# yassram/iterative-closest-point

Measured on AMD Instinct MI355X. Metric: ICP iterations/sec (synthetic 1048576-point pair, C4, exact NN), higher is better.
Workload: dtype f64 (30 exact fp64 grid searches (fp32 screen, candidates decided in fp64: the first from cell seeds, the seeded ones the fused grid iteration nn_grid_iter2_kernel, 75% of its queries kept their correspondence by the exclusion certificate without a walk); fp64 transform and reductions)

## Files before the change

### iterative-closest-point_amd/csrc/icp_grid.hip

```cpp
#include <hip/hip_runtime.h>

#include <algorithm>
#include <cmath>
#include <cstdlib>
#include <string>

#include "icp_canon.h"
#include "icp_device.h"
#include "icp_gridbox.h"
#include "icp_kernels.h"

namespace icp {
namespace {

__device__ __forceinline__ double d64g(double px, double py, double pz, double mx, double my,
                                       double mz)
{
    const double dx = px - mx;
    const double dy = py - my;
    const double dz = pz - mz;
    return (dx * dx + dy * dy) + dz * dz;
}


__global__ __launch_bounds__(kBlock) void grid_keys_kernel(const double *__restrict__ mx, const double *__restrict__ my,
                                                         const double *__restrict__ mz, int nm, GridView gv,
                                                         unsigned *__restrict__ key, int *__restrict__ val)
{
    const int i = blockIdx.x * kBlock + threadIdx.x;
    if (i >= nm) return;
    const int cx = cell1(mx[i], gv.lo[0], gv.inv_h, gv.g[0]);
    const int cy = cell1(my[i], gv.lo[1], gv.inv_h, gv.g[1]);
    const int cz = cell1(mz[i], gv.lo[2], gv.inv_h, gv.g[2]);
    key[i] = (unsigned)((cz * gv.g[1] + cy) * gv.g[0] + cx);
    val[i] = i;
}

__global__ __launch_bounds__(kBlock) void grid_starts_kernel(const unsigned *__restrict__ skey, int nm, int ncell,
                                                           int *__restrict__ start)
{
    const int c = blockIdx.x * kBlock + threadIdx.x;
    if (c > ncell) return;
    int lo = 0, hi = nm;
    while (lo < hi) {
        const int mid = (lo + hi) >> 1;
        if (skey[mid] < (unsigned)c) lo = mid + 1;
        else hi = mid;
    }
    start[c] = lo;
}

__global__ __launch_bounds__(kBlock) void grid_gather_kernel(const double4 *__restrict__ m4, int nm,
                                                           const int *__restrict__ sval, double4 *__restrict__ pts,
                                                           float4 *__restrict__ pts32, double c0, double c1, double c2)
{
    const int k = blockIdx.x * kBlock + threadIdx.x;
    if (k >= nm) return;
    const int i = sval[k];
// ... 438 lines not shown
                    const int r = r0 + u * G;
                    int a = 0, b = 0;
                    int x0 = c0[0], x1 = c1[0];
                    const int cy = c0[1] + r % ny, cz = c0[2] + r / ny;
                    if (r < nrows && (!trim || trim_row(q, best, gv, cy, cz, x0, x1))) {
                        const int row = (cz * gv.g[1] + cy) * gv.g[0];
                        a = gv.start[row + x0];
                        b = gv.start[row + x1 + 1];
                    }
                    k0[u] = a;
                    pre[u + 1] = pre[u] + (b - a);
                }
                const int total = pre[KR];
                for (int f0 = 0; f0 < total; f0 += KU) {
                    int k[KU];
#pragma unroll
                    for (int v = 0; v < KU; ++v) {
                        const int f = f0 + v;
                        int p = k0[0] + f;
#pragma unroll
                        for (int u = 1; u < KR; ++u)
                            if (f >= pre[u]) p = k0[u] + (f - pre[u]);
                        k[v] = f < total ? p : -1;
                    }
                    double4 m[KU];
#pragma unroll
                    for (int v = 0; v < KU; ++v)
                        if (k[v] >= 0) m[v] = gv.pts[k[v]];
#pragma unroll
                    for (int v = 0; v < KU; ++v)
                        if (k[v] >= 0)
                            lex_min_pos(best, bi, bk, d64g(q[0], q[1], q[2], m[v].x, m[v].y, m[v].z), (int)m[v].w,
                                        k[v]);
                }
            }
            group_lex_min_pos<G>(best, bi, bk);
            if (sub == 0) {
                const double4 w = bk >= 0 ? gv.pts[bk] : m4[bi];
                idx[t] = bi;
                yx[t] = w.x;
                yy[t] = w.y;
                yz[t] = w.z;
            }
        }
        const bool far = !ok && sub == 0;
        const int fs = wave_append(far_count, far);
        if (far) {
            far_list[fs] = t;
            far_hint[fs] = h;
        }
    }
}

__device__ __forceinline__ float seeded_bound32(double best, double e)
{
    const double s = sqrt(best) * (1.0 + 0x1.0p-50) + 1.7320508075688774 * e;
    return (float)(s * s * (1.0 + 0x1.0p-20)) * (1.0f + 0x1.0p-22f);
}

template <int G, int KR, int KU>
__global__ __launch_bounds__(kBlock) void nn_grid_seeded32_kernel(
    int n, const double *__restrict__ px, const double *__restrict__ py, const double *__restrict__ pz, GridView gv,
    int budget, const double *__restrict__ seedd, const double4 *__restrict__ m4, int *__restrict__ idx,
    double *__restrict__ yx, double *__restrict__ yy, double *__restrict__ yz, int *far_count,
    int *__restrict__ far_list, int *__restrict__ far_hint, const int *__restrict__ stop, int xcd_remap, int trim)
{
    if (stop && *stop) return;
    const int sub = threadIdx.x & (G - 1);
    const int groups = gridDim.x * (kBlock / G);
    const int bx = xcd_row((int)blockIdx.x, (int)gridDim.x, xcd_remap);
    for (int t = (bx * kBlock + threadIdx.x) / G; t < n; t += groups) {
        const int h = idx[t];
        const double q[3] = {px[t], py[t], pz[t]};
        double best = seedd[t];
        int bi = h, bk = -1, c0[3], c1[3];
        const bool ok = h >= 0 && best == best && best < INFINITY && complete_box(q, best, gv, budget, c0, c1);
        if (ok) {
            const double o0 = q[0] - gv.c32[0], o1 = q[1] - gv.c32[1], o2 = q[2] - gv.c32[2];
            const float q0 = (float)o0, q1 = (float)o1, q2 = (float)o2;
            const double e = std::ldexp(fmax(fabs(o0), fmax(fabs(o1), fabs(o2))), -23) + gv.em32;
            const float T = seeded_bound32(best, e);
            const int ny = c1[1] - c0[1] + 1;
            const int nrows = ny * (c1[2] - c0[2] + 1);
            for (int r0 = sub; r0 < nrows; r0 += KR * G) {
                int k0[KR], pre[KR + 1];
                pre[0] = 0;
#pragma unroll
                for (int u = 0; u < KR; ++u) {
                    const int r = r0 + u * G;
                    int a = 0, b = 0;
                    int x0 = c0[0], x1 = c1[0];
                    const int cy = c0[1] + r % ny, cz = c0[2] + r / ny;
                    if (r < nrows && (!trim || trim_row(q, best, gv, cy, cz, x0, x1))) {
                        const int row = (cz * gv.g[1] + cy) * gv.g[0];
                        a = gv.start[row + x0];
                        b = gv.start[row + x1 + 1];
                    }
                    k0[u] = a;
                    pre[u + 1] = pre[u] + (b - a);
                }
                const int total = pre[KR];
                for (int f0 = 0; f0 < total; f0 += KU) {
                    int k[KU];
#pragma unroll
                    for (int v = 0; v < KU; ++v) {
                        const int f = f0 + v;
                        int p = k0[0] + f;
#pragma unroll
                        for (int u = 1; u < KR; ++u)
                            if (f >= pre[u]) p = k0[u] + (f - pre[u]);
                        k[v] = f < total ? p : -1;
// ... 553 lines not shown
    __syncthreads();
    if (threadIdx.x < kCanonCols) {
        const int k = threadIdx.x;
        double v[4];
#pragma unroll
        for (int j = 0; j < 4; ++j)
            v[j] = H == 1 ? sh[j][k] : 0.0 + (sh[H * j][k] + sh[H * j + H - 1][k]);
        rows[(size_t)k * R + wr] = (v[0] + v[1]) + (v[2] + v[3]);
    }
    __shared__ int s_cnt[2][NW];
    for (int o = 32; o >= 1; o >>= 1) far += __shfl_xor(far, o, 64);
    if (lane == 0) {
        s_cnt[0][wave] = far;
        s_cnt[1][wave] = nbig;
    }
    __syncthreads();
    if (threadIdx.x < 2) {
        int tot = 0;
        for (int w = 0; w < NW; ++w) tot += s_cnt[threadIdx.x][w];
        int *dst = threadIdx.x == 0 ? far_acc : big_count;
        if (tot && dst) atomicAdd(dst, tot);
    }
}

constexpr int kNoBound = (int)0xbf800000u;
constexpr int kIter2Slot = 8;
constexpr int kIter2Tile = kCanonCols * kLeafStride;
static_assert(32 * kIter2Slot + 32 / 2 <= kIter2Tile, "the hand-off slots and the walker list alias the tiles");

#ifndef ICP_ITER2_DBG
#define ICP_ITER2_DBG 0
#endif
#ifndef ICP_ITER2_F64
#define ICP_ITER2_F64 0
#endif
#ifndef ICP_ITER2_KU
#define ICP_ITER2_KU 4
#endif
#ifndef ICP_ITER2_KR
#define ICP_ITER2_KR 3
#endif
#ifndef ICP_ITER2_KCAND
#define ICP_ITER2_KCAND ICP_ITER_KCAND
#endif
#ifndef ICP_ITER2_WAVES
#define ICP_ITER2_WAVES 4
#endif
#ifndef ICP_ITER2_GFLOOR
#define ICP_ITER2_GFLOOR 1
#endif
#ifndef ICP_ITER2_NWG_DEFAULT
#define ICP_ITER2_NWG_DEFAULT 1
#endif
template <int KR, int KU, int CH, int NWG>
__global__ __launch_bounds__(64 * NWG) __attribute__((amdgpu_waves_per_eu(ICP_ITER2_WAVES))) void nn_grid_iter2_kernel(
    int n, double *__restrict__ px, double *__restrict__ py, double *__restrict__ pz, double *__restrict__ yx,
    double *__restrict__ yy, double *__restrict__ yz, int *__restrict__ idx, const IterState *__restrict__ st,
    float4 *__restrict__ p32, GridView gv, int box, int budget, int nm, const double4 *__restrict__ m4,
    double *__restrict__ rows, int *far_acc, double far_d2, int *big_count, int xform, int xcd_l, CertArgs ca,
    unsigned long long *__restrict__ dbg)
{
    static_assert(CH == 1 || CH == 2, "one or two chunks a task");
    constexpr bool kDbg = ICP_ITER2_DBG != 0;
    unsigned long long dcnt[4] = {0, 0, 0, 0};
    static_assert(NWG == 4 || NWG == 1, "a row or a strand a workgroup");
    constexpr int NW = NWG, QL = 2 / CH;
    __shared__ double s_tile[NW][CH * kIter2Tile];
    if (st->done) return;
    const int lane = threadIdx.x & 63, wave = threadIdx.x >> 6, u = lane / QL, sub = lane % QL;
    const int C = canon_chunks((size_t)n), S = canon_strands((size_t)n), R = canon_rows((size_t)n);
    const int s = NWG == 4 ? xcd_row((int)blockIdx.x, R, xcd_l) * 4 + wave
                           : xcd_row((int)blockIdx.x, S, xcd_l > 0 ? 4 * xcd_l : xcd_l);
    const int wr = s >> 2;
    double *const tile = s_tile[wave];
    double *const slots = tile;
    int *const wl = (int *)(tile + 32 * CH * kIter2Slot);
    const bool cert_on = ca.state != nullptr, cert_in = cert_on && ca.valid != 0;
    auto wave_sync = [] {
        __builtin_amdgcn_fence(__ATOMIC_RELEASE, "wavefront");
        __builtin_amdgcn_wave_barrier();
        __builtin_amdgcn_fence(__ATOMIC_ACQUIRE, "wavefront");
    };
    double acc = 0.0;
    int far = 0, nbig = 0, ncert = 0, nwalk = 0;
    auto slot_t = [&](int c, int uu) { return (c + (uu >> 5) * S) * kCanonChunk + (uu & 31); };
    for (int c = s; s < S && c < C; c += CH * S) {
        const int t = slot_t(c, u);
        const bool active = c + (u >> 5) * S < C && t < n;
        if (kDbg) dcnt[0] += 1;
        double q[3] = {0.0, 0.0, 0.0}, y[3] = {0.0, 0.0, 0.0};
        int h = -1;
        int4 cs4 = make_int4(kNoBound, kNoBound, -1, -1);
        double mot = 0.0;
        if (active) {
            const double p0 = px[t], p1 = py[t], p2 = pz[t];
            y[0] = yx[t];
            y[1] = yy[t];
            y[2] = yz[t];
            h = idx[t];
            if (cert_in) cs4 = ca.state[t];
            if (xform) {
                transform_point(st->xf, p0, p1, p2, q[0], q[1], q[2]);
                if (cert_in)
                    mot = (double)(__builtin_amdgcn_sqrtf(__double2float_ru(residual2(p0, p1, p2, q[0], q[1], q[2]))) *
                                   (1.0f + 0x1.0p-21f));
            } else {
                q[0] = p0;
                q[1] = p1;
                q[2] = p2;
            }
        }
        const double e = active ? residual2(y[0], y[1], y[2], q[0], q[1], q[2]) : 0.0;
        if (active && sub == 0 && xform) {
            px[t] = q[0];
            py[t] = q[1];
            pz[t] = q[2];
            if (p32)
                p32[t] = make_float4((float)(q[0] - st->xf.c[0]), (float)(q[1] - st->xf.c[1]), (float)(q[2] - st->xf.c[2]),
                                     0.0f);
        }
        if (active && sub == 0) {
            if (far_d2 >= 0.0) {
                if (xform) far += e > far_d2 ? 1 : 0;
            } else if (!(h >= 0 && e * (gv.inv_h * gv.inv_h) < 2.2)) {
                int b0[3], b1[3];
                far += h >= 0 && e == e && e < INFINITY && complete_box(q, e, gv, box, b0, b1) ? 0 : 1;
            }
        }
        double best = e;
        int bi = h;
        double w[3] = {y[0], y[1], y[2]};
        bool certd = false;
        const float R1 = __int_as_float(cs4.x), R3 = __int_as_float(cs4.y);
        if (cert_in && active && h >= 0 && (R1 > 0.0f || R3 > 0.0f)) {
            const double R1c = ((double)R1 - mot) - (double)R1 * 0x1.0p-48;
            const double R3c = ((double)R3 - mot) - (double)R3 * 0x1.0p-48;
            auto inside = [](double d2, double r) { return r > 0.0 && d2 * (1.0 + 0x1.0p-38) < r * r * (1.0 - 0x1.0p-50); };
            double R1n = R1c;
            int2 pn = make_int2(cs4.z, cs4.w);
            certd = inside(e, R1c);
            if (kDbg && !certd && ca.two && cs4.w >= 0 && R3c > 0.0) dcnt[3] += 1;
            if (!certd && ca.two && cs4.w >= 0 && R3c > 0.0) {
                const double4 r2 = gv.pts[cs4.w];
                const double d2 = d64g(q[0], q[1], q[2], r2.x, r2.y, r2.z);
                const int mi2 = (int)r2.w;
                const bool swap = d2 < e || (d2 == e && (unsigned)mi2 < (unsigned)h);
                const double db = swap ? d2 : e;
                if (inside(db, R3c)) {
                    certd = true;
                    const double lb = fmin(R3c, sqrt(swap ? e : d2) * (1.0 - 0x1.0p-40));
                    if (swap) {
                        best = d2;
                        bi = mi2;
                        w[0] = r2.x;
                        w[1] = r2.y;
                        w[2] = r2.z;
                        R1n = lb;
                        pn = make_int2(cs4.w, cs4.z);
                    } else {
                        R1n = fmax(R1c, lb);
                    }
                }
            }
            if (certd && sub == 0) {
                const int4 ns = make_int4(__float_as_int(R1n > 0.0 ? __double2float_rd(R1n) : -1.0f),
                                          __float_as_int(R3c > 0.0 ? __double2float_rd(R3c) : -1.0f), pn.x, pn.y);
                if (bi != h) {
                    ca.state[t] = ns;
                    idx[t] = bi;
                    yx[t] = w[0];
                    yy[t] = w[1];
                    yz[t] = w[2];
                } else {
                    *(int2 *)&ca.state[t] = make_int2(ns.x, ns.y);
                }
            }
        }
        double *const sl = slots + u * kIter2Slot;
        const bool walker = active && !certd;
        if (walker && sub == 0) {
            sl[0] = q[0];
            sl[1] = q[1];
            sl[2] = q[2];
            sl[3] = best;
            ((int *)(sl + 7))[0] = bi;
            ((int *)(sl + 7))[1] = h;
        }
        if (active && sub == 0) {
            sl[4] = w[0];
            sl[5] = w[1];
            sl[6] = w[2];
        }
        const unsigned long long wm = __ballot(walker && sub == 0);
        ncert += certd && sub == 0 ? 1 : 0;
        nwalk += walker && sub == 0 ? 1 : 0;
        const int nW = __popcll(wm);
        if (walker && sub == 0) wl[__popcll(wm & ((1ull << lane) - 1ull))] = u;
        wave_sync();
        if (kDbg) dcnt[1] += nW;
        for (int b0 = 0; b0 < nW; b0 += 32) {
            if (kDbg) dcnt[2] += 1;
            const int nb = min(32, nW - b0);
            const int lg = nb > 16 ? 1 : nb > 8 ? 2 : nb > 4 ? 3 : nb > 2 ? 4 : nb > 1 ? 5 : 6;
            const int G = ICP_ITER2_GFLOOR ? 64 / nb : 1 << lg;
            const int ginv = (65536 + G - 1) / G;
            const int wi = (lane * ginv) >> 16, ws = lane - wi * G, gbase = wi * G;
            const bool wact = wi < nb;
            const int wu = wl[b0 + (wact ? wi : 0)];
            const double *const ws_sl = slots + wu * kIter2Slot;
            double wq[3], wb = INFINITY;
            int wbi = -1;
            wq[0] = ws_sl[0];
            wq[1] = ws_sl[1];
            wq[2] = ws_sl[2];
            if (wact) {
                wb = ws_sl[3];
                wbi = ((const int *)(ws_sl + 7))[0];
            }
            int c0[3] = {0, 0, 0}, c1[3] = {-1, -1, -1};
            double ew = wb;
            bool ok = false;
            if (wact && wbi >= 0 && wb == wb && wb < INFINITY) {
                if (cert_on) {
                    const double rs = sqrt(wb) + ca.skin;
                    ew = rs * rs;
                    ok = complete_box(wq, ew, gv, box, c0, c1);
                    if (!ok) ew = wb;
                }
                if (!ok) ok = complete_box(wq, ew, gv, box, c0, c1);
            }
            if (wact && ws == 0) slots[wu * kIter2Slot + 3] = ew;
            int bk = -1;
            float a1 = INFINITY, a2 = INFINITY;
            int k1 = -1;
            auto other = [&](float v, int k) {
                const bool lt = v < a1;
                a2 = __builtin_amdgcn_fmed3f(a1, v, a2);
                a1 = lt ? v : a1;
                k1 = lt ? k : k1;
            };
            auto eq_of = [&]() {
                const double o0 = wq[0] - gv.c32[0], o1 = wq[1] - gv.c32[1], o2 = wq[2] - gv.c32[2];
                return std::ldexp(fmax(fabs(o0), fmax(fabs(o1), fabs(o2))), -23) + gv.em32;
            };
            if (ok) {
                const float f0 = (float)(wq[0] - gv.c32[0]), f1 = (float)(wq[1] - gv.c32[1]), f2 = (float)(wq[2] - gv.c32[2]);
                const double eq = eq_of();
                const float T = seeded_bound32(wb, eq);
                const int ny = c1[1] - c0[1] + 1, nrq = ny * (c1[2] - c0[2] + 1);
                constexpr int kCand = ICP_ITER2_KCAND;
                int cand[kCand], nc = 0;
                auto flush = [&]() {
                    double4 r[kCand];
#pragma unroll
                    for (int j = 0; j < kCand; ++j)
                        if (j < nc) r[j] = gv.pts[cand[j]];
#pragma unroll
                    for (int j = 0; j < kCand; ++j) {
                        if (j >= nc) break;
                        const int mi = (int)r[j].w;
                        const double d = d64g(wq[0], wq[1], wq[2], r[j].x, r[j].y, r[j].z);
                        if (d < wb || (d == wb && (unsigned)mi < (unsigned)wbi)) {
                            if (cert_on && bk >= 0) other(__double2float_rd(wb), bk);
                            wb = d;
                            wbi = mi;
                            bk = cand[j];
                        } else if (cert_on) {
                            other(__double2float_rd(d), cand[j]);
                        }
                    }
                    nc = 0;
                };
                auto test = [&](const float4 (&m)[KU], const int (&kk)[KU]) {
                    bool cnd[KU];
                    bool anyc = false;
#pragma unroll
                    for (int v = 0; v < KU; ++v) {
                        const float dx = f0 - m[v].x, dy = f1 - m[v].y, dz = f2 - m[v].z;
                        const float d32 = (dx * dx + dy * dy) + dz * dz;
                        const bool val = kk[v] >= 0, fr = d32 > T;
                        if (cert_on) other(val && fr ? d32 : INFINITY, kk[v]);
                        const bool self = val && !fr && __float_as_int(m[v].w) == wbi;
                        bk = self ? kk[v] : bk;
                        cnd[v] = val && !fr && !self;
                        anyc = anyc || cnd[v];
                    }
                    if (__ballot(anyc)) {
#pragma unroll
                        for (int v = 0; v < KU; ++v)
                            if (cnd[v]) {
                                cand[nc++] = kk[v];
                                if (nc == kCand) flush();
                            }
                    }
                };
                const float inv_ny = 1.0f / (float)ny;
                float tr[3];
#pragma unroll
                for (int a = 0; a < 3; ++a) tr[a] = (float)((wq[a] - gv.lo[a]) * gv.inv_h - (double)c0[a]);
                const float rcf = (float)(sqrt(ew) * gv.inv_h * (1.0 + 0x1.0p-18) +
                                          0x1.0p-20 * (1.0 + fabs((double)tr[0]) + fabs((double)tr[1]) + fabs((double)tr[2])));
                const float rc2 = rcf * rcf, xroom = 0x1.0p-20f * (1.0f + fabsf(tr[0]));
                const float xspan = (float)(c1[0] - c0[0] + 1);
                auto row_run = [&](int r, int &a0, int &a1r) {
                    a0 = 0;
                    a1r = 0;
                    if (r >= nrq) return;
                    const int rz = (int)(((float)r + 0.5f) * inv_ny), ry = r - rz * ny;
                    const int row = ((c0[2] + rz) * gv.g[1] + c0[1] + ry) * gv.g[0];
                    int x0 = c0[0], x1 = c1[0];
                    const float dy = fmaxf(0.0f, fmaxf((float)ry - tr[1], tr[1] - (float)(ry + 1)));
                    const float dz = fmaxf(0.0f, fmaxf((float)rz - tr[2], tr[2] - (float)(rz + 1)));
                    const float rem = rc2 - dy * dy - dz * dz;
                    if (rem < 0.0f) return;
                    const float xw = __builtin_amdgcn_sqrtf(rem) * (1.0f + 0x1.0p-20f) + xroom;
                    x0 = max(x0, c0[0] + (int)floorf(fmaxf(tr[0] - xw, -1.0f)));
                    x1 = min(x1, c0[0] + (int)floorf(fminf(tr[0] + xw, xspan)));
                    if (x0 <= x1) {
                        a0 = gv.start[row + x0];
                        a1r = gv.start[row + x1 + 1];
                    }
                };
                {
                    for (int r0 = ws; r0 < nrq; r0 += KR * G) {
                        int k0[KR], pre[KR + 1];
                        pre[0] = 0;
#pragma unroll
                        for (int v = 0; v < KR; ++v) {
                            int a0, a1r;
                            row_run(r0 + v * G, a0, a1r);
                            k0[v] = a0;
                            pre[v + 1] = pre[v] + (a1r - a0);
                        }
                        const int tot = pre[KR];
                        for (int f0 = 0; f0 < tot; f0 += KU) {
                            int kk[KU];
#pragma unroll
                            for (int v = 0; v < KU; ++v) {
                                const int f = f0 + v;
                                int pp = k0[0] + f;
#pragma unroll
                                for (int x = 1; x < KR; ++x)
                                    if (f >= pre[x]) pp = k0[x] + (f - pre[x]);
                                kk[v] = f < tot ? pp : -1;
                            }
                            if constexpr (ICP_ITER2_F64) {
                                double4 mm[KU];
#pragma unroll
                                for (int v = 0; v < KU; ++v) mm[v] = gv.pts[kk[v] >= 0 ? kk[v] : 0];
#pragma unroll
                                for (int v = 0; v < KU; ++v) {
                                    const double d = d64g(wq[0], wq[1], wq[2], mm[v].x, mm[v].y, mm[v].z);
                                    const int mi = (int)mm[v].w, kv = kk[v];
                                    const bool val = kv >= 0, self = val && mi == wbi;
                                    const bool win = val && !self && (d < wb || (d == wb && (unsigned)mi < (unsigned)wbi));
                                    if (cert_on) {
                                        const float ov = win ? (bk >= 0 ? (float)wb * 0x1.fffffcp-1f : INFINITY)
                                                             : (val && !self ? (float)d * 0x1.fffffcp-1f : INFINITY);
                                        other(ov, win ? bk : kv);
                                    }
                                    wb = win ? d : wb;
                                    wbi = win ? mi : wbi;
                                    bk = win || self ? kv : bk;
                                }
                            } else {
                                float4 mm[KU];
#pragma unroll
                                for (int v = 0; v < KU; ++v) mm[v] = gv.pts32[kk[v] >= 0 ? kk[v] : 0];
                                test(mm, kk);
                            }
                        }
                    }
                }
                if constexpr (!ICP_ITER2_F64)
                    if (nc) flush();
            }
            for (int o = 1; o < G; o <<= 1) {
                const int pw = ws ^ o;
                const bool pin = pw < G;
                const int pl = gbase + (pin ? pw : ws);
                const double ob = pin ? __shfl(wb, pl, 64) : INFINITY;
                const int oi = pin ? __shfl(wbi, pl, 64) : -1, ok2 = pin ? __shfl(bk, pl, 64) : -1;
                const bool theirs = ob < wb || (ob == wb && (unsigned)oi < (unsigned)wbi);
                if (cert_on) {
                    const float oa1 = pin ? __shfl(a1, pl, 64) : INFINITY, oa2 = pin ? __shfl(a2, pl, 64) : INFINITY;
                    const int ok1 = pin ? __shfl(k1, pl, 64) : -1;
                    if (a1 <= oa1) {
                        a2 = fminf(a2, oa1);
                    } else {
                        a2 = fminf(oa2, a1);
                        a1 = oa1;
                        k1 = ok1;
                    }
                    if (oi != wbi) {
                        const int lk = theirs ? bk : ok2;
                        if (lk >= 0) other((float)(theirs ? wb : ob) * 0x1.fffffcp-1f, lk);
                    }
                }
                if (theirs) {
                    wb = ob;
                    wbi = oi;
                    bk = ok2;
                } else if (ob == wb && oi == wbi) {
                    bk = max(bk, ok2);
                }
            }
            unsigned long long bigm = __ballot(wact && ws == 0 && !ok);
            nbig += __popcll(bigm);
            bool whole = false;
            while (bigm) {
                const int bl = __ffsll((long long)bigm) - 1;
                bigm &= bigm - 1;
                const double bq[3] = {__shfl(wq[0], bl, 64), __shfl(wq[1], bl, 64), __shfl(wq[2], bl, 64)};
                const double be = __shfl(wb, bl, 64);
                const int bh = __shfl(wbi, bl, 64);
                double b2 = INFINITY;
                int bj = -1;
                int d0[3], d1[3];
                if (bh >= 0 && be == be && be < INFINITY && complete_box(bq, be, gv, budget, d0, d1)) {
                    b2 = be;
                    bj = bh;
                    scan_box<64>(bq, d0, d1, gv, lane, b2, bj);
                } else {
                    for (int k = lane; k < nm; k += 64) {
                        const double4 m = m4[k];
                        lex_min(b2, bj, d64g(bq[0], bq[1], bq[2], m.x, m.y, m.z), k);
                    }
                }
                group_lex_min<64>(b2, bj);
                if (wi == ((bl * ginv) >> 16)) {
                    wb = b2;
                    wbi = bj < 0 ? 0 : bj;
                    whole = true;
                }
            }
            if (wact && ws == 0) {
                double *const rs_sl = slots + wu * kIter2Slot;
                const int seed = ((const int *)(rs_sl + 7))[0], wh = ((const int *)(rs_sl + 7))[1];
                const int wt = slot_t(c, wu);
                if (wbi != seed) {
                    const double4 m = whole ? m4[wbi] : gv.pts[bk];
                    rs_sl[4] = m.x;
                    rs_sl[5] = m.y;
                    rs_sl[6] = m.z;
                }
                if (wbi != wh) {
                    idx[wt] = wbi;
                    yx[wt] = rs_sl[4];
                    yy[wt] = rs_sl[5];
                    yz[wt] = rs_sl[6];
                }
                if (cert_on) {
                    int4 ns = make_int4(kNoBound, kNoBound, -1, -1);
                    if (ok && !whole && bk >= 0) {
                        const double u0 = sqrt(rs_sl[3]) * (1.0 - 0x1.0p-40);
                        const double ec = ICP_ITER2_F64 ? 0.0 : 1.7320508075688774 * eq_of() * (1.0 + 0x1.0p-20);
                        auto lower = [&](float a) {
                            return a < INFINITY ? fmin(u0, sqrt((double)a) * (1.0 - 0x1.0p-20) - ec) : u0;
                        };
                        const double r1 = lower(a1), r3 = ca.two ? lower(a2) : -1.0;
                        ns = make_int4(__float_as_int(r1 > 0.0 ? __double2float_rd(r1) : -1.0f),
                                       __float_as_int(r3 > 0.0 ? __double2float_rd(r3) : -1.0f), bk, ca.two ? k1 : -1);
                    }
                    ca.state[wt] = ns;
                }
            }
            wave_sync();
        }
        if (active) {
            y[0] = sl[4];
            y[1] = sl[5];
            y[2] = sl[6];
        }
        wave_sync();
        const double cp[3] = {st->shift_p[0], st->shift_p[1], st->shift_p[2]};
        const double cy[3] = {st->shift_y[0], st->shift_y[1], st->shift_y[2]};
        const double d[6] = {active ? q[0] - cp[0] : 0.0, active ? q[1] - cp[1] : 0.0, active ? q[2] - cp[2] : 0.0,
                             active ? y[0] - cy[0] : 0.0, active ? y[1] - cy[1] : 0.0, active ? y[2] - cy[2] : 0.0};
        double *const lf = tile + (u >> 5) * kIter2Tile;
#pragma unroll
        for (int k = 0; k < kCanonCols; ++k) {
            double leaf;
            if (k < 6) leaf = 0.0 + d[k];
            else if (k < 15) leaf = 0.0 + d[(k - 6) / 3] * d[3 + (k - 6) % 3];
            else if (k == 15) leaf = 0.0 + ((d[3] * d[3] + d[4] * d[4]) + d[5] * d[5]);
            else if (k == 16) leaf = 0.0 + ((d[0] * d[0] + d[1] * d[1]) + d[2] * d[2]);
            else leaf = active ? 0.0 + e : 0.0;
            if (!active) leaf = 0.0;
            if (sub == 0) lf[k * kLeafStride + (u & 31)] = leaf;
        }
        wave_sync();
        double tv = 0.0;
        if ((lane & 31) < kCanonCols && (CH == 2 || lane < 32)) {
            const double *col = tile + (lane >> 5) * kIter2Tile + (lane & 31) * kLeafStride;
            double part[4];
#pragma unroll
            for (int g8 = 0; g8 < 4; ++g8) {
                double v[8];
#pragma unroll
                for (int j = 0; j < 8; ++j) v[j] = col[8 * g8 + j];
                part[g8] = ((v[0] + v[1]) + (v[2] + v[3])) + ((v[4] + v[5]) + (v[6] + v[7]));
            }
            tv = (part[0] + part[1]) + (part[2] + part[3]);
        }
        const double tb = CH == 2 ? __shfl(tv, (lane & 31) + 32, 64) : 0.0;
        if (lane < kCanonCols) {
            acc = acc + tv;
            if (CH == 2 && c + S < C) acc = acc + tb;
        }
        wave_sync();
    }
    if (kDbg && dbg && lane == 0)
        for (int f = 0; f < 4; ++f)
            if (dcnt[f]) atomicAdd(dbg + f, dcnt[f]);
    if constexpr (NWG == 4) {
        __shared__ double sh[NW][kCanonCols];
        if (lane < kCanonCols) sh[wave][lane] = acc;
        __syncthreads();
        if (threadIdx.x < kCanonCols) {
            const int k = threadIdx.x;
            rows[(size_t)k * R + wr] = (sh[0][k] + sh[1][k]) + (sh[2][k] + sh[3][k]);
        }
    } else if (s < S && lane < kCanonCols) {
        rows[(size_t)lane * S + s] = acc;
    }
    __shared__ int s_cnt[4][NW];
    for (int o = 32; o >= 1; o >>= 1) {
        far += __shfl_xor(far, o, 64);
        ncert += __shfl_xor(ncert, o, 64);
        nwalk += __shfl_xor(nwalk, o, 64);
    }
    if (lane == 0) {
        s_cnt[0][wave] = far;
        s_cnt[1][wave] = nbig;
        s_cnt[2][wave] = ncert;
        s_cnt[3][wave] = nwalk;
    }
    __syncthreads();
    if (threadIdx.x < 4) {
        int tot = 0;
        for (int w = 0; w < NW; ++w) tot += s_cnt[threadIdx.x][w];
        if (threadIdx.x < 2) {
            int *dst = threadIdx.x == 0 ? far_acc : big_count;
            if (tot && dst) atomicAdd(dst, tot);
        } else if (ca.counts && (NWG == 4 || s < S)) {
            ca.counts[2 * (NWG == 4 ? wr : s) + (threadIdx.x - 2)] += (unsigned long long)tot;
        }
    }
}

}

bool launch_nn_grid_iter(int n, double *px, double *py, double *pz, double *yx, double *yy, double *yz, int *idx,
                         const IterState *st_dev, float4 *p32, const GridView &gv, int box, int budget, int nm,
                         const double4 *m4, double *rows, int *far_acc, double far_d2, int *big_count, hipStream_t st,
                         unsigned long long *dbg, int xform, const CertArgs &ca, int *strands)
{
    if (strands) *strands = 0;
    if (n <= 0) return false;
    static const bool stage = [] {
        const char *e = getenv("ICP_ITER_STAGE");
        return e && atoi(e) == 1;
    }();
    static const bool wide_on = [] {
        const char *e = getenv("ICP_ITER_WIDE");
        return e && atoi(e) == 1;
    }();
    const int R = canon_rows((size_t)n);
    static const int xcd_env = [] {
        const char *e = getenv("ICP_ITER_XCD_L");
        return e ? atoi(e) : -2;
    }();
    const int xcd_l = xcd_env != -2 ? xcd_env : (canon_chunks((size_t)n) >= 8192 ? 32 : -1);
    static const bool v2 = [] {
        const char *e = getenv("ICP_ITER_V2");
        return !(e && e[0] == '0');
    }();
    if (v2 && !stage && !(wide_on && n <= kIterWideMax) && (!dbg || ICP_ITER2_DBG)) {
        static const int ch = [] {
            const char *e = getenv("ICP_ITER2_CH");
            return e && atoi(e) == 1 ? 1 : 2;
        }();
        static const int nwg = [] {
            const char *e = getenv("ICP_ITER2_NWG");
            return e && atoi(e) == 4 ? 4 : ICP_ITER2_NWG_DEFAULT;
        }();
        const int S = canon_strands((size_t)n);
        if (strands) *strands = nwg == 1 ? S : 0;
        if (ch == 2 && nwg == 1)
            nn_grid_iter2_kernel<ICP_ITER2_KR, ICP_ITER2_KU, 2, 1><<<S, 64, 0, st>>>(
                n, px, py, pz, yx, yy, yz, idx, st_dev, p32, gv, box, budget, nm, m4, rows, far_acc, far_d2, big_count,
                xform, xcd_l, ca, dbg);
        else if (ch == 2)
            nn_grid_iter2_kernel<ICP_ITER2_KR, ICP_ITER2_KU, 2, 4><<<R, kBlock, 0, st>>>(
                n, px, py, pz, yx, yy, yz, idx, st_dev, p32, gv, box, budget, nm, m4, rows, far_acc, far_d2, big_count,
                xform, xcd_l, ca, dbg);
        else if (nwg == 1)
            nn_grid_iter2_kernel<ICP_ITER2_KR, ICP_ITER2_KU, 1, 1><<<S, 64, 0, st>>>(
                n, px, py, pz, yx, yy, yz, idx, st_dev, p32, gv, box, budget, nm, m4, rows, far_acc, far_d2, big_count,
                xform, xcd_l, ca, dbg);
        else
            nn_grid_iter2_kernel<ICP_ITER2_KR, ICP_ITER2_KU, 1, 4><<<R, kBlock, 0, st>>>(
                n, px, py, pz, yx, yy, yz, idx, st_dev, p32, gv, box, budget, nm, m4, rows, far_acc, far_d2, big_count,
                xform, xcd_l, ca, dbg);
        return ca.state != nullptr;
    }
    if (!stage && wide_on && n <= kIterWideMax)
        nn_grid_iter_kernel<false, 4><<<R, 2 * kBlock, 0, st>>>(n, px, py, pz, yx, yy, yz, idx, st_dev, p32, gv, box,
                                                                 budget, nm, m4, rows, far_acc, far_d2, big_count, dbg, xform, xcd_l);
    else if (stage)
        nn_grid_iter_kernel<true, 2><<<R, kBlock, 0, st>>>(n, px, py, pz, yx, yy, yz, idx, st_dev, p32, gv, box,
                                                            budget, nm, m4, rows, far_acc, far_d2, big_count, dbg, xform, xcd_l);
    else
        nn_grid_iter_kernel<false, 2><<<R, kBlock, 0, st>>>(n, px, py, pz, yx, yy, yz, idx, st_dev, p32, gv, box,
                                                             budget, nm, m4, rows, far_acc, far_d2, big_count, dbg, xform, xcd_l);
    return false;
}

namespace {
}

GridParams grid_params(const double *m_xyz, size_t nm)
{
    double lo[3] = {INFINITY, INFINITY, INFINITY}, hi[3] = {-INFINITY, -INFINITY, -INFINITY};
    for (size_t j = 0; j < nm; ++j)
        for (int a = 0; a < 3; ++a) {
            lo[a] = std::min(lo[a], m_xyz[3 * j + a]);
            hi[a] = std::max(hi[a], m_xyz[3 * j + a]);
        }
    return grid_params_box(lo, hi, nm);
}

GridParams grid_params_box(const double lo[3], const double hi[3], size_t nm)
{
    GridParams p{};
    double ext[3], emax = 0.0;
    for (int a = 0; a < 3; ++a) {
        ext[a] = hi[a] - lo[a];
        emax = std::max(emax, ext[a]);
        p.lo[a] = lo[a];
        p.c32[a] = lo[a] + 0.5 * ext[a];
    }
    p.em32 = std::isfinite(emax) ? std::ldexp(emax, -23) : INFINITY;
    if (!(emax > 0.0) || !std::isfinite(emax)) {
        p.g[0] = p.g[1] = p.g[2] = 1;
        p.inv_h = 1.0;
        return p;
    }
    static const double ppc = [] {
        const char *e = getenv("ICP_GRID_PPC");
        const double v = e ? atof(e) : 0.0;
        return v > 0.0 ? v : 2.0;
    }();
    double vol = 1.0;
    for (int a = 0; a < 3; ++a) vol *= std::max(ext[a], emax * 1e-3);
    double h = std::cbrt(vol * ppc / (double)std::max<size_t>(nm, 1));
    auto dims = [&](double hh, int g[3]) {
// ... 309 lines not shown
```

### iterative-closest-point_amd/csrc/icp_gridbox.h

```cpp
#pragma once
#include <hip/hip_runtime.h>

#include "icp_kernels.h"

namespace icp {

__device__ __forceinline__ int cellt(double t, int g)
{
    if (!(t > 0.0)) return 0;
    if (t >= (double)(g - 1)) return g - 1;
    return (int)t;
}

__device__ __forceinline__ int cell1(double x, double lo, double inv_h, int g)
{
    return cellt((x - lo) * inv_h, g);
}

__device__ __forceinline__ bool complete_box(const double q[3], double r2, const GridView &gv, int budget,
                                             int c0[3], int c1[3])
{
    const double R = sqrt(r2);
    long long cells = 1;
#pragma unroll
    for (int a = 0; a < 3; ++a) {
        const double s = (fabs(q[a]) + R) * 0x1.0p-44;
        c0[a] = cell1(q[a] - (R + s), gv.lo[a], gv.inv_h, gv.g[a]);
        c1[a] = cell1(q[a] + (R + s), gv.lo[a], gv.inv_h, gv.g[a]);
        cells *= (long long)(c1[a] - c0[a] + 1);
    }
    return cells <= budget;
}

__device__ __forceinline__ bool seed_far(const SeedArgs &sa, double q0, double q1, double q2, double d2)
{
    if (sa.far_box <= 0) return d2 > sa.far_d2;
    const double q[3] = {q0, q1, q2};
    int c0[3], c1[3];
    return !(d2 == d2 && d2 < INFINITY && complete_box(q, d2, sa.far_gv, sa.far_box, c0, c1));
}

}
```

Baseline: 9631.

## Pack iter2 kernel args into kernarg struct and use 32-bit address offsets

The fused grid iteration kernel now takes a single argument struct and re-reads fields from the kernarg segment through scalar pointers at each use. The intent is to keep pointers and constants in SGPRs instead of holding them in VGPRs across the loop. A template flag chooses unsigned 32-bit byte offsets for indexing when sizes allow, which cuts 64-bit address arithmetic. It also carries the radius instead of its square so several fp64 sqrts drop out, and swaps some fp64 sqrts for fp32 sqrt with looser bounds. The cost is more template variants, and the certificate lower bounds become slightly looser, so fewer queries may be certified.

Result: faster. 10190 (median of 6 runs) (+5.8%).

```diff
diff --git a/iterative-closest-point_amd/csrc/icp_grid.hip b/iterative-closest-point_amd/csrc/icp_grid.hip
--- a/iterative-closest-point_amd/csrc/icp_grid.hip
+++ b/iterative-closest-point_amd/csrc/icp_grid.hip
@@ -4,6 +4,7 @@
 #include <cmath>
 #include <cstdlib>
 #include <string>
+#include <type_traits>
 
 #include "icp_canon.h"
 #include "icp_device.h"
@@ -548,11 +549,12 @@
     }
 }
 
-__device__ __forceinline__ float seeded_bound32(double best, double e)
-{
-    const double s = sqrt(best) * (1.0 + 0x1.0p-50) + 1.7320508075688774 * e;
+__device__ __forceinline__ float seeded_bound32_root(double root, double e)
+{
+    const double s = root * (1.0 + 0x1.0p-50) + 1.7320508075688774 * e;
     return (float)(s * s * (1.0 + 0x1.0p-20)) * (1.0f + 0x1.0p-22f);
 }
+__device__ __forceinline__ float seeded_bound32(double best, double e) { return seeded_bound32_root(sqrt(best), e); }
 
 template <int G, int KR, int KU>
 __global__ __launch_bounds__(kBlock) void nn_grid_seeded32_kernel(
@@ -1212,13 +1214,47 @@
 #ifndef ICP_ITER2_NWG_DEFAULT
 #define ICP_ITER2_NWG_DEFAULT 1
 #endif
-template <int KR, int KU, int CH, int NWG>
+struct Iter2Args {
+    int n;
+    double *px, *py, *pz, *yx, *yy, *yz;
+    int *idx;
+    const IterState *st;
+    float4 *p32;
+    GridView gv;
+    int box, budget, nm;
+    const double4 *m4;
+    double *rows;
+    int *far_acc;
+    double far_d2;
+    int *big_count;
+    int xform, xcd_l;
+    CertArgs ca;
+    unsigned long long *dbg;
+};
+static_assert(std::is_trivially_copyable<Iter2Args>::value, "passed by value in the kernel-argument segment");
+#define ICP_CONST_AS __attribute__((address_space(4)))
+__device__ __forceinline__ const Iter2Args &iter2_args()
+{
+    auto *p = (const ICP_CONST_AS Iter2Args *)__builtin_amdgcn_kernarg_segment_ptr();
+    asm volatile("" : "+s"(p));
+    return *(const Iter2Args *)p;
+}
+__device__ __forceinline__ const IterState &iter2_state(const IterState *st)
+{
+    auto *p = (const ICP_CONST_AS IterState *)st;
+    asm volatile("" : "+s"(p));
+    return *(const IterState *)p;
+}
+
+template <bool A32, class T> __device__ __forceinline__ T &at32(T *b, int i)
+{
+    if constexpr (A32) return *(T *)((char *)b + (unsigned)i * (unsigned)sizeof(T));
+    else return b[i];
+}
+
+template <int KR, int KU, int CH, int NWG, bool A32>
 __global__ __launch_bounds__(64 * NWG) __attribute__((amdgpu_waves_per_eu(ICP_ITER2_WAVES))) void nn_grid_iter2_kernel(
-    int n, double *__restrict__ px, double *__restrict__ py, double *__restrict__ pz, double *__restrict__ yx,
-    double *__restrict__ yy, double *__restrict__ yz, int *__restrict__ idx, const IterState *__restrict__ st,
-    float4 *__restrict__ p32, GridView gv, int box, int budget, int nm, const double4 *__restrict__ m4,
-    double *__restrict__ rows, int *far_acc, double far_d2, int *big_count, int xform, int xcd_l, CertArgs ca,
-    unsigned long long *__restrict__ dbg)
+    Iter2Args args_)
 {
     static_assert(CH == 1 || CH == 2, "one or two chunks a task");
     constexpr bool kDbg = ICP_ITER2_DBG != 0;
@@ -1226,7 +1262,10 @@
     static_assert(NWG == 4 || NWG == 1, "a row or a strand a workgroup");
     constexpr int NW = NWG, QL = 2 / CH;
     __shared__ double s_tile[NW][CH * kIter2Tile];
-    if (st->done) return;
+    const Iter2Args &T = iter2_args();
+    const IterState *const st = T.st;
+    if (iter2_state(st).done) return;
+    const int n = T.n, xcd_l = T.xcd_l, xform = T.xform;
     const int lane = threadIdx.x & 63, wave = threadIdx.x >> 6, u = lane / QL, sub = lane % QL;
     const int C = canon_chunks((size_t)n), S = canon_strands((size_t)n), R = canon_rows((size_t)n);
     const int s = NWG == 4 ? xcd_row((int)blockIdx.x, R, xcd_l) * 4 + wave
@@ -1235,7 +1274,8 @@
     double *const tile = s_tile[wave];
     double *const slots = tile;
     int *const wl = (int *)(tile + 32 * CH * kIter2Slot);
-    const bool cert_on = ca.state != nullptr, cert_in = cert_on && ca.valid != 0;
+    auto at = [](auto *b, int i) -> auto & { return at32<A32>(b, i); };
+    const bool cert_on = T.ca.state != nullptr, cert_in = cert_on && T.ca.valid != 0, two = T.ca.two != 0;
     auto wave_sync = [] {
         __builtin_amdgcn_fence(__ATOMIC_RELEASE, "wavefront");
         __builtin_amdgcn_wave_barrier();
@@ -1248,19 +1288,26 @@
         const int t = slot_t(c, u);
         const bool active = c + (u >> 5) * S < C && t < n;
         if (kDbg) dcnt[0] += 1;
+        const Iter2Args &A = iter2_args();
+        const Xform xf = iter2_state(st).xf;
+        double *const px = A.px, *const py = A.py, *const pz = A.pz, *const yx = A.yx, *const yy = A.yy, *const yz = A.yz;
+        int *const idx = A.idx;
+        int4 *const cstate = A.ca.state;
+        float4 *const p32 = A.p32;
+        const double far_d2 = A.far_d2;
         double q[3] = {0.0, 0.0, 0.0}, y[3] = {0.0, 0.0, 0.0};
         int h = -1;
         int4 cs4 = make_int4(kNoBound, kNoBound, -1, -1);
         double mot = 0.0;
         if (active) {
-            const double p0 = px[t], p1 = py[t], p2 = pz[t];
-            y[0] = yx[t];
-            y[1] = yy[t];
-            y[2] = yz[t];
-            h = idx[t];
-            if (cert_in) cs4 = ca.state[t];
+            const double p0 = at(px, t), p1 = at(py, t), p2 = at(pz, t);
+            y[0] = at(yx, t);
+            y[1] = at(yy, t);
+            y[2] = at(yz, t);
+            h = at(idx, t);
+            if (cert_in) cs4 = at(cstate, t);
             if (xform) {
-                transform_point(st->xf, p0, p1, p2, q[0], q[1], q[2]);
+                transform_point(xf, p0, p1, p2, q[0], q[1], q[2]);
                 if (cert_in)
                     mot = (double)(__builtin_amdgcn_sqrtf(__double2float_ru(residual2(p0, p1, p2, q[0], q[1], q[2]))) *
                                    (1.0f + 0x1.0p-21f));
@@ -1272,19 +1319,19 @@
         }
         const double e = active ? residual2(y[0], y[1], y[2], q[0], q[1], q[2]) : 0.0;
         if (active && sub == 0 && xform) {
-            px[t] = q[0];
-            py[t] = q[1];
-            pz[t] = q[2];
+            at(px, t) = q[0];
+            at(py, t) = q[1];
+            at(pz, t) = q[2];
             if (p32)
-                p32[t] = make_float4((float)(q[0] - st->xf.c[0]), (float)(q[1] - st->xf.c[1]), (float)(q[2] - st->xf.c[2]),
+                at(p32, t) = make_float4((float)(q[0] - xf.c[0]), (float)(q[1] - xf.c[1]), (float)(q[2] - xf.c[2]),
                                      0.0f);
         }
         if (active && sub == 0) {
             if (far_d2 >= 0.0) {
                 if (xform) far += e > far_d2 ? 1 : 0;
-            } else if (!(h >= 0 && e * (gv.inv_h * gv.inv_h) < 2.2)) {
+            } else if (!(h >= 0 && e * (A.gv.inv_h * A.gv.inv_h) < 2.2)) {
                 int b0[3], b1[3];
-                far += h >= 0 && e == e && e < INFINITY && complete_box(q, e, gv, box, b0, b1) ? 0 : 1;
+                far += h >= 0 && e == e && e < INFINITY && complete_box(q, e, A.gv, A.box, b0, b1) ? 0 : 1;
             }
         }
         double best = e;
@@ -1299,16 +1346,16 @@
             double R1n = R1c;
             int2 pn = make_int2(cs4.z, cs4.w);
             certd = inside(e, R1c);
-            if (kDbg && !certd && ca.two && cs4.w >= 0 && R3c > 0.0) dcnt[3] += 1;
-            if (!certd && ca.two && cs4.w >= 0 && R3c > 0.0) {
-                const double4 r2 = gv.pts[cs4.w];
+            if (kDbg && !certd && two && cs4.w >= 0 && R3c > 0.0) dcnt[3] += 1;
+            if (!certd && two && cs4.w >= 0 && R3c > 0.0) {
+                const double4 r2 = at(A.gv.pts, cs4.w);
                 const double d2 = d64g(q[0], q[1], q[2], r2.x, r2.y, r2.z);
                 const int mi2 = (int)r2.w;
                 const bool swap = d2 < e || (d2 == e && (unsigned)mi2 < (unsigned)h);
                 const double db = swap ? d2 : e;
                 if (inside(db, R3c)) {
                     certd = true;
-                    const double lb = fmin(R3c, sqrt(swap ? e : d2) * (1.0 - 0x1.0p-40));
+                    const double lb = fmin(R3c, (double)__builtin_amdgcn_sqrtf(__double2float_rd(swap ? e : d2)) * (1.0 - 0x1.0p-21));
                     if (swap) {
                         best = d2;
                         bi = mi2;
@@ -1326,13 +1373,13 @@
                 const int4 ns = make_int4(__float_as_int(R1n > 0.0 ? __double2float_rd(R1n) : -1.0f),
                                           __float_as_int(R3c > 0.0 ? __double2float_rd(R3c) : -1.0f), pn.x, pn.y);
                 if (bi != h) {
-                    ca.state[t] = ns;
-                    idx[t] = bi;
-                    yx[t] = w[0];
-                    yy[t] = w[1];
-                    yz[t] = w[2];
+                    at(cstate, t) = ns;
+                    at(idx, t) = bi;
+                    at(yx, t) = w[0];
+                    at(yy, t) = w[1];
+                    at(yz, t) = w[2];
                 } else {
-                    *(int2 *)&ca.state[t] = make_int2(ns.x, ns.y);
+                    *(int2 *)&at(cstate, t) = make_int2(ns.x, ns.y);
                 }
             }
         }
@@ -1359,6 +1406,10 @@
         wave_sync();
         if (kDbg) dcnt[1] += nW;
         for (int b0 = 0; b0 < nW; b0 += 32) {
+            const Iter2Args &D = iter2_args();
+            const GridView gv = D.gv;
+            const int box = D.box;
+            const double skin = D.ca.skin;
             if (kDbg) dcnt[2] += 1;
             const int nb = min(32, nW - b0);
             const int lg = nb > 16 ? 1 : nb > 8 ? 2 : nb > 4 ? 3 : nb > 2 ? 4 : nb > 1 ? 5 : 6;
@@ -1378,18 +1429,21 @@
                 wbi = ((const int *)(ws_sl + 7))[0];
             }
             int c0[3] = {0, 0, 0}, c1[3] = {-1, -1, -1};
-            double ew = wb;
+            double rw = 0.0, rb = 0.0, s0 = 0.0;
             bool ok = false;
             if (wact && wbi >= 0 && wb == wb && wb < INFINITY) {
+                s0 = sqrt(wb);
                 if (cert_on) {
-                    const double rs = sqrt(wb) + ca.skin;
-                    ew = rs * rs;
-                    ok = complete_box(wq, ew, gv, box, c0, c1);
-                    if (!ok) ew = wb;
-                }
-                if (!ok) ok = complete_box(wq, ew, gv, box, c0, c1);
-            }
-            if (wact && ws == 0) slots[wu * kIter2Slot + 3] = ew;
+                    rw = s0 + skin;
+                    rb = rw * (1.0 + 0x1.0p-51);
+                    ok = complete_box_r(wq, rb, gv, box, c0, c1);
+                }
+                if (!ok) {
+                    rw = rb = s0;
+                    ok = complete_box_r(wq, rb, gv, box, c0, c1);
+                }
+            }
+            if (wact && ws == 0) slots[wu * kIter2Slot + 3] = rw;
             int bk = -1;
             float a1 = INFINITY, a2 = INFINITY;
             int k1 = -1;
@@ -1403,10 +1457,11 @@
                 const double o0 = wq[0] - gv.c32[0], o1 = wq[1] - gv.c32[1], o2 = wq[2] - gv.c32[2];
                 return std::ldexp(fmax(fabs(o0), fmax(fabs(o1), fabs(o2))), -23) + gv.em32;
             };
+            double eq = 0.0;
             if (ok) {
                 const float f0 = (float)(wq[0] - gv.c32[0]), f1 = (float)(wq[1] - gv.c32[1]), f2 = (float)(wq[2] - gv.c32[2]);
-                const double eq = eq_of();
-                const float T = seeded_bound32(wb, eq);
+                eq = eq_of();
+                const float T = seeded_bound32_root(s0, eq);
                 const int ny = c1[1] - c0[1] + 1, nrq = ny * (c1[2] - c0[2] + 1);
                 constexpr int kCand = ICP_ITER2_KCAND;
                 int cand[kCand], nc = 0;
@@ -1414,7 +1469,7 @@
                     double4 r[kCand];
 #pragma unroll
                     for (int j = 0; j < kCand; ++j)
-                        if (j < nc) r[j] = gv.pts[cand[j]];
+                        if (j < nc) r[j] = at(gv.pts, cand[j]);
 #pragma unroll
                     for (int j = 0; j < kCand; ++j) {
                         if (j >= nc) break;
@@ -1458,7 +1513,7 @@
                 float tr[3];
 #pragma unroll
                 for (int a = 0; a < 3; ++a) tr[a] = (float)((wq[a] - gv.lo[a]) * gv.inv_h - (double)c0[a]);
-                const float rcf = (float)(sqrt(ew) * gv.inv_h * (1.0 + 0x1.0p-18) +
+                const float rcf = (float)(rb * gv.inv_h * (1.0 + 0x1.0p-18) +
                                           0x1.0p-20 * (1.0 + fabs((double)tr[0]) + fabs((double)tr[1]) + fabs((double)tr[2])));
                 const float rc2 = rcf * rcf, xroom = 0x1.0p-20f * (1.0f + fabsf(tr[0]));
                 const float xspan = (float)(c1[0] - c0[0] + 1);
@@ -1477,8 +1532,8 @@
                     x0 = max(x0, c0[0] + (int)floorf(fmaxf(tr[0] - xw, -1.0f)));
                     x1 = min(x1, c0[0] + (int)floorf(fminf(tr[0] + xw, xspan)));
                     if (x0 <= x1) {
-                        a0 = gv.start[row + x0];
-                        a1r = gv.start[row + x1 + 1];
+                        a0 = at(gv.start, row + x0);
+                        a1r = at(gv.start, row + x1 + 1);
                     }
                 };
                 {
@@ -1507,7 +1562,7 @@
                             if constexpr (ICP_ITER2_F64) {
                                 double4 mm[KU];
 #pragma unroll
-                                for (int v = 0; v < KU; ++v) mm[v] = gv.pts[kk[v] >= 0 ? kk[v] : 0];
+                                for (int v = 0; v < KU; ++v) mm[v] = at(gv.pts, kk[v] >= 0 ? kk[v] : 0);
 #pragma unroll
                                 for (int v = 0; v < KU; ++v) {
                                     const double d = d64g(wq[0], wq[1], wq[2], mm[v].x, mm[v].y, mm[v].z);
@@ -1526,7 +1581,7 @@
                             } else {
                                 float4 mm[KU];
 #pragma unroll
-                                for (int v = 0; v < KU; ++v) mm[v] = gv.pts32[kk[v] >= 0 ? kk[v] : 0];
+                                for (int v = 0; v < KU; ++v) mm[v] = at(gv.pts32, kk[v] >= 0 ? kk[v] : 0);
                                 test(mm, kk);
                             }
                         }
@@ -1571,19 +1626,20 @@
             while (bigm) {
                 const int bl = __ffsll((long long)bigm) - 1;
                 bigm &= bigm - 1;
+                const Iter2Args &B = iter2_args();
                 const double bq[3] = {__shfl(wq[0], bl, 64), __shfl(wq[1], bl, 64), __shfl(wq[2], bl, 64)};
                 const double be = __shfl(wb, bl, 64);
                 const int bh = __shfl(wbi, bl, 64);
                 double b2 = INFINITY;
                 int bj = -1;
                 int d0[3], d1[3];
-                if (bh >= 0 && be == be && be < INFINITY && complete_box(bq, be, gv, budget, d0, d1)) {
+                if (bh >= 0 && be == be && be < INFINITY && complete_box(bq, be, B.gv, B.budget, d0, d1)) {
                     b2 = be;
                     bj = bh;
-                    scan_box<64>(bq, d0, d1, gv, lane, b2, bj);
+                    scan_box<64>(bq, d0, d1, B.gv, lane, b2, bj);
                 } else {
-                    for (int k = lane; k < nm; k += 64) {
-                        const double4 m = m4[k];
+                    for (int k = lane; k < B.nm; k += 64) {
+                        const double4 m = B.m4[k];
                         lex_min(b2, bj, d64g(bq[0], bq[1], bq[2], m.x, m.y, m.z), k);
                     }
                 }
@@ -1595,34 +1651,39 @@
                 }
             }
             if (wact && ws == 0) {
+                const Iter2Args &O = iter2_args();
+                int *const o_idx = O.idx;
+                double *const o_yx = O.yx, *const o_yy = O.yy, *const o_yz = O.yz;
+                int4 *const o_state = O.ca.state;
+                const double4 *const o_pts = O.gv.pts;
                 double *const rs_sl = slots + wu * kIter2Slot;
                 const int seed = ((const int *)(rs_sl + 7))[0], wh = ((const int *)(rs_sl + 7))[1];
                 const int wt = slot_t(c, wu);
                 if (wbi != seed) {
-                    const double4 m = whole ? m4[wbi] : gv.pts[bk];
+                    const double4 m = whole ? at(O.m4, wbi) : at(o_pts, bk);
                     rs_sl[4] = m.x;
                     rs_sl[5] = m.y;
                     rs_sl[6] = m.z;
                 }
                 if (wbi != wh) {
-                    idx[wt] = wbi;
-                    yx[wt] = rs_sl[4];
-                    yy[wt] = rs_sl[5];
-                    yz[wt] = rs_sl[6];
+                    at(o_idx, wt) = wbi;
+                    at(o_yx, wt) = rs_sl[4];
+                    at(o_yy, wt) = rs_sl[5];
+                    at(o_yz, wt) = rs_sl[6];
                 }
                 if (cert_on) {
                     int4 ns = make_int4(kNoBound, kNoBound, -1, -1);
                     if (ok && !whole && bk >= 0) {
-                        const double u0 = sqrt(rs_sl[3]) * (1.0 - 0x1.0p-40);
-                        const double ec = ICP_ITER2_F64 ? 0.0 : 1.7320508075688774 * eq_of() * (1.0 + 0x1.0p-20);
+                        const double u0 = rs_sl[3] * (1.0 - 0x1.0p-40);
+                        const double ec = ICP_ITER2_F64 ? 0.0 : 1.7320508075688774 * eq * (1.0 + 0x1.0p-20);
                         auto lower = [&](float a) {
-                            return a < INFINITY ? fmin(u0, sqrt((double)a) * (1.0 - 0x1.0p-20) - ec) : u0;
+                            return a < INFINITY ? fmin(u0, (double)__builtin_amdgcn_sqrtf(a) * (1.0 - 0x1.0p-20) - ec) : u0;
                         };
-                        const double r1 = lower(a1), r3 = ca.two ? lower(a2) : -1.0;
+                        const double r1 = lower(a1), r3 = two ? lower(a2) : -1.0;
                         ns = make_int4(__float_as_int(r1 > 0.0 ? __double2float_rd(r1) : -1.0f),
-                                       __float_as_int(r3 > 0.0 ? __double2float_rd(r3) : -1.0f), bk, ca.two ? k1 : -1);
+                                       __float_as_int(r3 > 0.0 ? __double2float_rd(r3) : -1.0f), bk, two ? k1 : -1);
                     }
-                    ca.state[wt] = ns;
+                    at(o_state, wt) = ns;
                 }
             }
             wave_sync();
@@ -1633,8 +1694,9 @@
             y[2] = sl[6];
         }
         wave_sync();
-        const double cp[3] = {st->shift_p[0], st->shift_p[1], st->shift_p[2]};
-        const double cy[3] = {st->shift_y[0], st->shift_y[1], st->shift_y[2]};
+        const IterState &sg = iter2_state(st);
+        const double cp[3] = {sg.shift_p[0], sg.shift_p[1], sg.shift_p[2]};
+        const double cy[3] = {sg.shift_y[0], sg.shift_y[1], sg.shift_y[2]};
         const double d[6] = {active ? q[0] - cp[0] : 0.0, active ? q[1] - cp[1] : 0.0, active ? q[2] - cp[2] : 0.0,
                              active ? y[0] - cy[0] : 0.0, active ? y[1] - cy[1] : 0.0, active ? y[2] - cy[2] : 0.0};
         double *const lf = tile + (u >> 5) * kIter2Tile;
@@ -1646,7 +1708,6 @@
             else if (k == 15) leaf = 0.0 + ((d[3] * d[3] + d[4] * d[4]) + d[5] * d[5]);
             else if (k == 16) leaf = 0.0 + ((d[0] * d[0] + d[1] * d[1]) + d[2] * d[2]);
             else leaf = active ? 0.0 + e : 0.0;
-            if (!active) leaf = 0.0;
             if (sub == 0) lf[k * kLeafStride + (u & 31)] = leaf;
         }
         wave_sync();
@@ -1670,6 +1731,8 @@
         }
         wave_sync();
     }
+    const Iter2Args &E = iter2_args();
+    unsigned long long *const dbg = E.dbg;
     if (kDbg && dbg && lane == 0)
         for (int f = 0; f < 4; ++f)
             if (dcnt[f]) atomicAdd(dbg + f, dcnt[f]);
@@ -1679,10 +1742,10 @@
         __syncthreads();
         if (threadIdx.x < kCanonCols) {
             const int k = threadIdx.x;
-            rows[(size_t)k * R + wr] = (sh[0][k] + sh[1][k]) + (sh[2][k] + sh[3][k]);
+            E.rows[(size_t)k * R + wr] = (sh[0][k] + sh[1][k]) + (sh[2][k] + sh[3][k]);
         }
     } else if (s < S && lane < kCanonCols) {
-        rows[(size_t)lane * S + s] = acc;
+        E.rows[(size_t)lane * S + s] = acc;
     }
     __shared__ int s_cnt[4][NW];
     for (int o = 32; o >= 1; o >>= 1) {
@@ -1701,12 +1764,18 @@
         int tot = 0;
         for (int w = 0; w < NW; ++w) tot += s_cnt[threadIdx.x][w];
         if (threadIdx.x < 2) {
-            int *dst = threadIdx.x == 0 ? far_acc : big_count;
+            int *dst = threadIdx.x == 0 ? E.far_acc : E.big_count;
             if (tot && dst) atomicAdd(dst, tot);
-        } else if (ca.counts && (NWG == 4 || s < S)) {
-            ca.counts[2 * (NWG == 4 ? wr : s) + (threadIdx.x - 2)] += (unsigned long long)tot;
-        }
-    }
+        } else if (E.ca.counts && (NWG == 4 || s < S)) {
+            E.ca.counts[2 * (NWG == 4 ? wr : s) + (threadIdx.x - 2)] += (unsigned long long)tot;
+        }
+    }
+}
+
+bool iter2_addr32(int n, int nm, const GridView &gv)
+{
+    const long long ncell = (long long)gv.g[0] * gv.g[1] * gv.g[2];
+    return n <= (1 << 28) && nm <= (1 << 27) && ncell < (1ll << 30);
 }
 
 }
@@ -1747,22 +1816,29 @@
         }();
         const int S = canon_strands((size_t)n);
         if (strands) *strands = nwg == 1 ? S : 0;
-        if (ch == 2 && nwg == 1)
-            nn_grid_iter2_kernel<ICP_ITER2_KR, ICP_ITER2_KU, 2, 1><<<S, 64, 0, st>>>(
-                n, px, py, pz, yx, yy, yz, idx, st_dev, p32, gv, box, budget, nm, m4, rows, far_acc, far_d2, big_count,
-                xform, xcd_l, ca, dbg);
-        else if (ch == 2)
-            nn_grid_iter2_kernel<ICP_ITER2_KR, ICP_ITER2_KU, 2, 4><<<R, kBlock, 0, st>>>(
-                n, px, py, pz, yx, yy, yz, idx, st_dev, p32, gv, box, budget, nm, m4, rows, far_acc, far_d2, big_count,
-                xform, xcd_l, ca, dbg);
-        else if (nwg == 1)
-            nn_grid_iter2_kernel<ICP_ITER2_KR, ICP_ITER2_KU, 1, 1><<<S, 64, 0, st>>>(
-                n, px, py, pz, yx, yy, yz, idx, st_dev, p32, gv, box, budget, nm, m4, rows, far_acc, far_d2, big_count,
-                xform, xcd_l, ca, dbg);
-        else
-            nn_grid_iter2_kernel<ICP_ITER2_KR, ICP_ITER2_KU, 1, 4><<<R, kBlock, 0, st>>>(
-                n, px, py, pz, yx, yy, yz, idx, st_dev, p32, gv, box, budget, nm, m4, rows, far_acc, far_d2, big_count,
-                xform, xcd_l, ca, dbg);
+        const Iter2Args ka{n,      px, py, pz,   yx,      yy,     yz,        idx,   st_dev, p32, gv, box,
+                           budget, nm, m4, rows, far_acc, far_d2, big_count, xform, xcd_l,  ca,  dbg};
+        static const bool a32_on = [] {
+            const char *e = getenv("ICP_ITER2_A32");
+            return !(e && e[0] == '0');
+        }();
+        const bool a32 = a32_on && iter2_addr32(n, nm, gv);
+        auto launch = [&](auto chc, auto nwgc, auto a32c) {
+            constexpr int kCh = decltype(chc)::value, kNwg = decltype(nwgc)::value;
+            nn_grid_iter2_kernel<ICP_ITER2_KR, ICP_ITER2_KU, kCh, kNwg, decltype(a32c)::value>
+                <<<kNwg == 1 ? S : R, 64 * kNwg, 0, st>>>(ka);
+        };
+        auto with_a32 = [&](auto chc, auto nwgc) {
+            if (a32) launch(chc, nwgc, std::true_type{});
+            else launch(chc, nwgc, std::false_type{});
+        };
+        using I1 = std::integral_constant<int, 1>;
+        using I2 = std::integral_constant<int, 2>;
+        using I4 = std::integral_constant<int, 4>;
+        if (ch == 2 && nwg == 1) with_a32(I2{}, I1{});
+        else if (ch == 2) with_a32(I2{}, I4{});
+        else if (nwg == 1) with_a32(I1{}, I1{});
+        else with_a32(I1{}, I4{});
         return ca.state != nullptr;
     }
     if (!stage && wide_on && n <= kIterWideMax)
diff --git a/iterative-closest-point_amd/csrc/icp_gridbox.h b/iterative-closest-point_amd/csrc/icp_gridbox.h
--- a/iterative-closest-point_amd/csrc/icp_gridbox.h
+++ b/iterative-closest-point_amd/csrc/icp_gridbox.h
@@ -17,10 +17,9 @@
     return cellt((x - lo) * inv_h, g);
 }
 
-__device__ __forceinline__ bool complete_box(const double q[3], double r2, const GridView &gv, int budget,
-                                             int c0[3], int c1[3])
+__device__ __forceinline__ bool complete_box_r(const double q[3], double R, const GridView &gv, int budget,
+                                               int c0[3], int c1[3])
 {
-    const double R = sqrt(r2);
     long long cells = 1;
 #pragma unroll
     for (int a = 0; a < 3; ++a) {
@@ -32,6 +31,12 @@
     return cells <= budget;
 }
 
+__device__ __forceinline__ bool complete_box(const double q[3], double r2, const GridView &gv, int budget,
+                                             int c0[3], int c1[3])
+{
+    return complete_box_r(q, sqrt(r2), gv, budget, c0, c1);
+}
+
 __device__ __forceinline__ bool seed_far(const SeedArgs &sa, double q0, double q1, double q2, double d2)
 {
     if (sa.far_box <= 0) return d2 > sa.far_d2;
```
